# JuliaGraphics/Hikari.jl

Hardware: AMD Instinct MI355X
Metric: Mrays/s (higher is better)
Workload: dtype f32

## Files before the change

hikari.jl_amd/csrc/hk_ctx.cpp:

```cpp
#include "hk_host.h"

thread_local std::string g_err;
SlabCache g_slabs;

namespace hk {
static thread_local const Knobs* tl_knobs = nullptr;
const char* knob(const char* name) {
    if (!tl_knobs) return nullptr;
    auto it = tl_knobs->kv.find(name);
    return it == tl_knobs->kv.end() ? nullptr : it->second.c_str();
}
static const char* const KNOB_NAMES[] = {
    "HK_BATCH_PATHS_M", "HK_BVH_LEAF", "HK_BVH_BINS", "HK_QNODES", "HK_DEBUG_ALLOC", "HK_DELTA_ADVANCE", "HK_DYNAMIC_SEGMENTS", "HK_GREY", "HK_GREY_COMPACT", "HK_GREY_FLAT", "HK_MAX_PATHS_M",
    "HK_MID_LISTS", "HK_MID_PASS_PATHS_M", "HK_NODE_CACHE", "HK_NVDB_DENSE_MB", "HK_OVERLAP", "HK_PIPELINE", "HK_PIPELINE_AFTER", "HK_PIPELINE_MAX_PATHS_M", "HK_PRESELECT",
    "HK_SELECT_MIN_IDLE", "HK_SHADOW_FEED_ROUNDS", "HK_SHADOW_TRACK_BATCH", "HK_SMALL_PASS", "HK_SMALL_PASS_WAVES", "HK_SOBOL_LO_GB", "HK_SOBOL_TABLE_ONLY",
    "HK_STATE_CACHE_GB", "HK_STATE_SLAB", "HK_TICKET_SHARE", "HK_TRACK_ADVANCE", "HK_TRACK_EXTRA_ADVANCE", "HK_TRACK_MIN_PENDING", "HK_TRACK_POOL", "HK_TRACK_REFILL_IDLE",
    "HK_WALK_POOL", "HK_WALK_REFILL_IDLE", "HK_WALK_SPLIT", "HK_WAVES_PER_CU", "HK_READBACK_PIN", "HK_DEFER_EXTERNAL", "HK_SELECT_POOL", "HK_SMALL_PASS_FUSED", "HK_SMALL_PASS_MERGED", "HK_OCC_SCALE", "HK_ESCAPED_UNROLL", "HK_SHADOW_FINAL", "HK_TRI_PACK", "HK_LEAN_RECORDS", "HK_VIEW_CACHE", "HK_MAJORANT_BLOCK_VOXELS", "HK_BVH_BUILD_SMALL"};
static bool known_knob(const char* name) {
    for (const char* k : KNOB_NAMES)
        if (std::strcmp(k, name) == 0) return true;
    return false;
}
}
KnobScope::KnobScope(const hk::Knobs* k) : prev(hk::tl_knobs) { hk::tl_knobs = k; }
KnobScope::~KnobScope() { hk::tl_knobs = prev; }

void quiesce(hk_ctx* c) {
    if (!c) return;
    (void)hipStreamSynchronize(c->stream);
    if (c->aux) (void)hipStreamSynchronize(c->aux);
    for (auto& l : c->lanes)
        if (l.stream) (void)hipStreamSynchronize(l.stream);
}
int join_lanes(hk_ctx* c) {
    if (!c) return HK_OK;
    if (int e = flush_pending(c)) return e;
    if (!c->lanes_dirty) return HK_OK;
    for (auto& l : c->lanes)
        if (l.done) HIP_TRY(hipStreamWaitEvent(c->stream, l.done, 0));
    c->lanes_dirty = false;
    c->film_chain = false;
    if (c->have_span) HIP_TRY(hipEventRecord(c->ev_end, c->stream));
    return HK_OK;
}
hipEvent_t get_event(hk_ctx* c) {
    if (!c->event_pool.empty()) {
        hipEvent_t e = c->event_pool.back();
        c->event_pool.pop_back();
        return e;
    }
    hipEvent_t e;
    (void)hipEventCreate(&e);
    return e;
}
DCamera make_camera(const hk_camera& c) {
    DCamera d;
    std::memcpy(d.r2c, c.raster_to_camera, 64);
    std::memcpy(d.c2w, c.camera_to_world, 64);
    d.lens_radius = c.lens_radius;
    d.focal_distance = c.focal_distance;
    d.shutter_open = c.shutter_open;
    d.shutter_close = c.shutter_close;
    return d;
}

extern "C" const char* hk_last_error(void) { return g_err.c_str(); }

extern "C" int32_t hk_ctx_create(int32_t device_id, void* stream, hk_ctx** out) {
    if (!out) return fail(HK_ERR_INVALID, "out is null");
    int n = 0;
    HIP_TRY(hipGetDeviceCount(&n));
    if (device_id < 0 || device_id >= n) return fail(HK_ERR_INVALID, "bad device id");
    HIP_TRY(hipSetDevice(device_id));
    hk_ctx* c = new hk_ctx();
    c->device = device_id;
    c->stream = (hipStream_t)stream;
    hipDeviceProp_t prop;
    HIP_TRY(hipGetDeviceProperties(&prop, device_id));
    c->n_cu = prop.multiProcessorCount > 0 ? prop.multiProcessorCount : 256;
    c->own_stream_order = stream == nullptr;
    for (const char* name : hk::KNOB_NAMES)
        if (const char* e = std::getenv(name)) c->knobs.kv[name] = e;
    KnobScope knobs(&c->knobs);
    {
        c->waves_per_cu = hk::knob_int_in("HK_WAVES_PER_CU", 1, INT_MAX, 0);
        c->stat_rows = c->n_cu * 32 * 2;
        if (const char* e = hk::knob("HK_OVERLAP")) c->overlap = std::atoi(e) ? 1 : 0;
        else c->overlap = -1;
        if (const char* e = hk::knob("HK_STATE_CACHE_GB"))
            if (std::atol(e) >= 0) g_slabs.cap_bytes = (size_t)std::atol(e) << 30;
    }
    {
        std::vector<DStats> zero((size_t)c->stat_rows);
        std::memset(zero.data(), 0, zero.size() * sizeof(DStats));
        HIP_TRY(c->stats.upload(zero.data(), zero.size() * sizeof(DStats)));
    }
    HIP_TRY(hipEventCreate(&c->ev_begin));
    HIP_TRY(hipEventCreate(&c->ev_end));
    *out = c;
    return HK_OK;
// ... 266 lines not shown
```

hikari.jl_amd/csrc/hk_kernels.hip:

```cpp
#include <hip/hip_runtime.h>
#include <type_traits>
#include <cstdlib>
#include <cstdio>

#include "hikari_mi355x.h"
#include "hk_device.h"
#include "hk_edit_host.h"
#include "hk_bvh_decide.h"

using namespace hkd;

namespace {

__device__ __forceinline__ int lane_id() { return (int)(threadIdx.x & 63); }

struct WaveQ {
    uint32_t* base;
    int count;
};
__device__ __forceinline__ int global_wave() {
    const int w = (int)(threadIdx.x >> 6), b = (int)blockIdx.x;
    if (blockDim.x == 1024 && (gridDim.x & 7) == 0) return ((((b >> 3) * 4 + (w >> 2)) * 8 + (b & 7)) << 2) + (w & 3);
    if (blockDim.x == 512 && (gridDim.x & 7) == 0) return ((((b >> 3) * 2 + (w >> 2)) * 8 + (b & 7)) << 2) + (w & 3);
    return b * (int)(blockDim.x >> 6) + w;
// ... 2192 lines not shown
                        const int at = __popcll(dm & lt_mask);
                        pool[0][at] = e;
                        pool[1][at] = __float_as_uint(sp.x), pool[2][at] = __float_as_uint(sp.y), pool[3][at] = __float_as_uint(sp.z);
                        pool[4][at] = __float_as_uint(sn.x), pool[5][at] = __float_as_uint(sn.y), pool[6][at] = __float_as_uint(sn.z);
                        pool[7][at] = __float_as_uint(u_b);
                    }
                    pool_n = __popcll(dm);
                    __builtin_amdgcn_wave_barrier();
                }
            }
            const int avail = pool_n - pool_head;
            if (avail > 0) {
                const int rank = __popcll(free_m & lt_mask);
                if (!busy && rank < avail) {
                    const int at = pool_head + rank;
                    slot = pool[0][at];
                    p = mk3(__uint_as_float(pool[1][at]), __uint_as_float(pool[2][at]), __uint_as_float(pool[3][at]));
                    nn = mk3(__uint_as_float(pool[4][at]), __uint_as_float(pool[5][at]), __uint_as_float(pool[6][at]));
                    ub = __uint_as_float(pool[7][at]);
                    pmf = 1.0f - p_inf;
                    bits = root_bits, child = root_child;
                    lvl = 0;
                    busy = true;
                }
                const int free_n = __popcll(free_m);
                pool_head += free_n < avail ? free_n : avail;
            }
            if (__ballot(busy) == 0ull) {
                if (!more && pool_head == pool_n) break;
                continue;
            }
        }
        if (busy) {
            int res_light = -1;
            float res_pmf = 0.0f;
            if (lvl >= 64) {
                res_light = 0;
            } else {
                ++lvl;
                DLightNode n0, n1;
                if (NTOP > 0 && (int)child + 1 < n_top) {
                    n0 = lds_light_node<NTOP>(top, (int)child), n1 = lds_light_node<NTOP>(top, (int)child + 1);
                    asm volatile("" : "+v"(n0.bits));
                } else
                    n0 = load_light_node(sc.lnodes, (int)child), n1 = load_light_node(sc.lnodes, (int)child + 1);
                const float c0 = node_importance(n0, p, nn);
                const float c1 = node_importance(n1, p, nn);
                n_lnodes += 2;
                if (c0 == 0.0f && c1 == 0.0f) {
                    res_light = 0;
                } else {
                    const float p0 = c0 / (c0 + c1);
                    if (ub < p0) {
                        pmf *= p0;
                        ub = ub / p0;
                        bits = n0.bits, child = n0.child1_or_light;
                    } else {
                        pmf *= (1.0f - p0);
                        ub = (ub - p0) / (1.0f - p0);
                        bits = n1.bits, child = n1.child1_or_light;
                    }
                    if ((bits & 2u) && lvl < 64) {
                        res_light = (int)child;
                        res_pmf = pmf;
                    }
                }
            }
            if (res_light >= 0) {
                st.sel_light[slot] = make_uint2((uint32_t)res_light, __float_as_uint(res_pmf));
                busy = false;
            }
        }
    }
    stats += global_wave();
    wave_add(&stats->light_nodes, n_lnodes);
}

#ifndef HK_SHADE_WAVES_MATTE
#define HK_SHADE_WAVES_MATTE 4
#endif
#ifndef HK_SHADE_WAVES
#define HK_SHADE_WAVES 3
#endif
template <bool TWO_PLANES, bool SIMPLE>
HKD void shade_emission(const DPathState& st, const DPathGen& g, bool ones, const DScene& sc, const DTables& T, uint32_t slot, unsigned& n_lnodes, int depth, size_t seg) {
    const float4 H = st.hit[slot];
    const float4 O = ld_ray_o(st, g, slot, depth, seg), D = g.ray_d[slot];
    const v3 ro = mk3(O.x, O.y, O.z), rd = mk3(D.x, D.y, D.z);
    const float t_hit = H.x;
    const int prim = __float_as_int(H.y);
    const DTriMeta meta = tri_meta(sc, prim);
    if (meta.arealight <= 0) return;
    const Surface sf = surface_at(sc, prim, H.z, H.w, ro, rd, t_hit);
    const v3 wo = -rd;
    const uint2 pmeta = ld_meta(st, g, slot, depth);
    const S4 lambda = ld_lambda(st, g, slot, pmeta.y);
    const DLight& light = sc.lights[meta.arealight - 1];
    S4 Le = arealight_Le<TWO_PLANES, SIMPLE>(sc, T, light, wo, sf.n, sf.uv, lambda);
    if (is_black(Le)) return;
    const S4 beta = ld_throughput(g.beta, slot, ones), r_u = ld_ru(g, slot, ones, st.compact != 0), r_l = ld_rl(g, slot, ones, st.compact != 0);
    const uint32_t fl = pmeta.x;
    const int pdepth = (int)(fl & 0xff);
    const bool specular_bounce = (fl >> 8) & 1u;
    S4 contribution = beta * Le;
    S4 fin;
    if (pdepth == 0 || specular_bounce)
        fin = contribution / average(r_u);
    else {
        float choice = bvh_pmf(sc, sf.pi, sf.n, (int)meta.arealight, n_lnodes);
        float ct = fabsf(dot(sf.n, normalize(rd)));
        float light_pdf = 0.0f;
        if (ct > 0.0f && sf.area > 0.0f) light_pdf = choice * ((t_hit * t_hit) / (ct * sf.area));
        S4 rl = r_l * light_pdf;
        float den = average(r_u + rl);
        fin = den > 1e-10f ? contribution / den : contribution / average(r_u);
    }
    st4(&st.L[pmeta.y], ld4(&st.L[pmeta.y]) + fin);
}

template <int KIND>
struct ShadeWaves {
    static constexpr int value = (KIND == HK_MAT_COATED_DIFFUSE || KIND == HK_MAT_COATED_DIFFUSE_TRANSMISSION) ? 1 : (KIND == HK_MAT_MATTE ? HK_SHADE_WAVES_MATTE : HK_SHADE_WAVES);
};
#ifndef HK_SHADE_MIN_WAVES
#define HK_SHADE_MIN_WAVES 1
#endif
template <int KIND, bool SIMPLE, bool FT, bool PRE>
__device__ __forceinline__ void shade_body(const DPathState& st, const DScene& sc, const DTables& T, const DFrame& fr, const DSobol& sob, int depth, int first_kind, DStats* stats, const SegTickets& src,
                                           uint32_t* __restrict__ elist) {
    const int lane = lane_id();
    unsigned n_vertices = 0, n_lnodes = 0;
    HK_FOR_EACH_SEGMENT_FROM(gw, st, src) {
    const uint32_t* __restrict__ queue = st.mat_q + ((size_t)KIND * st.n_waves + gw) * st.wave_cap;
    const int n = *count_ptr(st, depth, Q_MAT0 + KIND, gw);
    const DPathGen g = gen_at(st, depth), gn = st.gen[(depth + 1) & 1];
    const size_t seg = (size_t)gw * st.wave_cap;
    const bool ones = depth == 0 && fr.implicit_ones;
    WavePos q_shadow{0}, q_next{0};
    if (!first_kind) {
        q_shadow.count = *count_ptr(st, depth, Q_SHADOW, gw);
        q_next.count = *count_ptr(st, depth + 1, Q_RAY, gw);
    }
    {
        int n_emit = 0;
        for (int base = 0; base < n || n_emit > 0; base += 64) {
            if (base < n) {
                const int i = base + lane;
                const uint32_t cand = i < n ? queue[i] : 0u;
                const bool em = i < n && (st.mat_id[cand] & HK_MAT_EMISSIVE_BIT) != 0;
                const unsigned long long m = __ballot(em);
                if (em) elist[n_emit + __popcll(m & ((1ull << lane) - 1ull))] = cand;
                n_emit += __popcll(m);
                if (n_emit < 64 && base + 64 < n) continue;
            }
            __builtin_amdgcn_fence(__ATOMIC_SEQ_CST, "wavefront");
            const int take = n_emit < 64 ? n_emit : 64;
            if (lane < take) shade_emission<KIND == HK_MAT_MATTE, SIMPLE>(st, g, ones, sc, T, elist[lane], n_lnodes, depth, seg);
            const int rest = n_emit - take;
            const uint32_t moved = lane < rest ? elist[64 + lane] : 0u;
            __builtin_amdgcn_fence(__ATOMIC_SEQ_CST, "wavefront");
            if (lane < rest) elist[lane] = moved;
            n_emit = rest;
        }
    }
    for (int base = 0; base < n; base += 64) {
        int i = base + lane;
        bool active = i < n;
        uint32_t slot = active ? queue[i] : 0u;
        bool push_shadow = false, push_ray = false;
        float4 H = make_float4(0, 0, 0, 0);
        Surface sf;
        v3 wo = mk3(0, 0, 1);
        DTriMeta meta{0u, 0u, 0u};
        S4 lambda = s4(0.0f), beta = s4(0.0f), r_u = s4(0.0f), kd_matte = s4(0.0f);
        uint32_t fl = 0, pslot = 0;
        int pdepth = 0, medium = -1;
        bool any_non_specular = false;
        SobolCtx sctx;
        const int base_dim = 6 + 7 * depth;
        float4 shO = make_float4(0, 0, 0, 0), shD = shO;
        S4 shLd = s4(0.0f), shRu = s4(0.0f), shRl = s4(0.0f);
        if (active) {
            ++n_vertices;
            H = stream_ld(&st.hit[slot]);
            float4 O = ld_ray_o(st, g, slot, depth, seg), D = stream_ld(&g.ray_d[slot]);
            v3 ro = mk3(O.x, O.y, O.z), rd = mk3(D.x, D.y, D.z);
            float t_hit = H.x;
            int prim = __float_as_int(H.y);
            sf = surface_at(sc, prim, H.z, H.w, ro, rd, t_hit);
            wo = -rd;
            meta = tri_meta(sc, prim);
            const uint2 pmeta = ld_meta(st, g, slot, depth);
            lambda = ld_lambda(st, g, slot, pmeta.y);
            if (ones)
                beta = s4(1.0f);
            else {
                const float4 bv = stream_ld(&g.beta[slot]);
                beta = s4(bv.x, bv.y, bv.z, bv.w);
            }
            r_u = ld_ru(g, slot, ones, st.compact != 0);
            fl = pmeta.x;
            pslot = pmeta.y;
            pdepth = (int)(fl & 0xff);
            any_non_specular = (fl >> 9) & 1u;
            medium = (int)(fl >> 16) - 1;

            int pix, k;
            split_slot(fr, pslot, pix, k);
            sctx = sobol_ctx_slot(sob, T.sobol, fr.x0, fr.y0, fr.tiles_x, pix, k, fr.first_sample + k * fr.sample_stride);

            if (KIND == HK_MAT_MATTE) kd_matte = matte_kd<SIMPLE>(sc, T, sc.materials[st.mat_id[slot] & ~HK_MAT_EMISSIVE_BIT], TexCtx(sf.uv, meta.prim_index, H.z, H.w), lambda);
#ifdef HK_ABLATE
            {
                float sink = 0.0f;
                if (HK_ABLATE == 1) {
                    uint32_t ps2 = pslot;
                    int d2 = base_dim;
                    asm volatile("" : "+v"(ps2));
                    asm volatile("" : "+s"(d2));
                    int pix2, k2;
                    split_slot(fr, ps2, pix2, k2);
                    SobolCtx c2 = sobol_ctx_slot(sob, T.sobol, fr.x0, fr.y0, fr.tiles_x, pix2, k2, fr.first_sample + k2 * fr.sample_stride);
                    v2 a = sobol_2d(c2, d2 + 3), b = sobol_2d(c2, d2 + 6);
                    sink = sobol_1d(c2, d2 + 1) + a.x + a.y + b.x + b.y + sobol_1d(c2, d2 + 7);
                }
                if (HK_ABLATE == 2 && sc.n_lights > 0) {
                    float u2 = H.z, pmf2;
                    asm volatile("" : "+v"(u2));
                    unsigned dummy = 0;
                    sink = (float)bvh_sample_light(sc, sf.pi, sf.ns, u2, pmf2, dummy) + pmf2;
                }
                if (HK_ABLATE == 3 && sc.n_lights > 0) {
                    uint32_t li = pslot;
                    asm volatile("" : "+v"(li));
                    LightSample l2 = sample_light(sc, T, sc.lights[li % (uint32_t)sc.n_lights], sf.pi, lambda, mk2(H.z, H.w));
                    sink = l2.pdf + l2.Li.x + l2.Li.w + l2.wi.x + l2.p_light.z;
                }
                if (HK_ABLATE == 4) {
                    S4 l2 = lambda;
                    asm volatile("" : "+v"(l2.x), "+v"(l2.y), "+v"(l2.z), "+v"(l2.w));
                    S4 k2 = matte_kd(sc, T, sc.materials[st.mat_id[slot] & ~HK_MAT_EMISSIVE_BIT], TexCtx(sf.uv, meta.prim_index, H.z, H.w), l2);
                    sink = k2.x + k2.y + k2.z + k2.w;
                }
                if (HK_ABLATE == 5) {
                    float b2 = H.z;
                    asm volatile("" : "+v"(b2));
                    Surface s2 = surface_at(sc, prim, b2, H.w, ro, rd, t_hit);
                    sink = s2.pi.x + s2.n.y + s2.ns.z + s2.uv.x + s2.area;
                }
                if (HK_ABLATE == 6) {
                    v3 w2 = wo;
                    asm volatile("" : "+v"(w2.x), "+v"(w2.y), "+v"(w2.z));
                    float p2;
                    S4 f2 = eval_matte_kd(kd_matte, w2, sf.n, sf.ns, p2);
                    BSDFSample s2 = sample_matte_kd(sc, sc.materials[st.mat_id[slot] & ~HK_MAT_EMISSIVE_BIT], kd_matte, w2, sf.ns, TexCtx(sf.uv, meta.prim_index, H.z, H.w), mk2(H.z, H.w));
                    sink = f2.x + f2.w + p2 + s2.pdf + s2.wi.x + s2.f.y;
                }
                asm volatile("" : : "v"(sink));
            }
#endif

            if (sc.n_lights > 0) {
                const DMaterial& mat = sc.materials[st.mat_id[slot] & ~HK_MAT_EMISSIVE_BIT];
                float light_pmf;
                int light_idx;
                if constexpr (PRE) {
                    const uint2 pre = st.sel_light[slot];
                    light_idx = (int)pre.x;
                    light_pmf = __uint_as_float(pre.y);
                } else {
                    float light_select = sobol_1d<FT>(sctx, base_dim + 1);
                    light_idx = bvh_sample_light(sc, sf.pi, sf.ns, light_select, light_pmf, n_lnodes);
                }
                if (light_idx >= 1 && light_idx <= sc.n_lights && light_pmf > 0.0f) {
                    const DLight& sel = sc.lights[light_idx - 1];
                    v2 u_light = mk2(0.0f, 0.0f);
                    if (sel.kind >= HK_LIGHT_AMBIENT) u_light = sobol_2d<FT>(sctx, base_dim + 3);
                    LightSample ls = sample_light<KIND == HK_MAT_MATTE, SIMPLE>(sc, T, sel, sf.pi, lambda, u_light);
                    if (ls.pdf > 0.0f && !is_black(ls.Li)) {
                        float bsdf_pdf;
                        S4 f = KIND == HK_MAT_MATTE ? eval_matte_kd(kd_matte, wo, ls.wi, sf.ns, bsdf_pdf)
                                                    : eval_bsdf<KIND>(sc, T, mat, wo, ls.wi, sf.ns, TexCtx(sf.uv, meta.prim_index, H.z, H.w), lambda, bsdf_pdf);
                        if (!is_black(f)) {
                            float ct = fabsf(dot(ls.wi, sf.ns));
                            S4 Ld = beta * f * ls.Li * ct;
                            if (!is_black(Ld)) {
                                v3 off = 1e-4f * sf.ns;
                                v3 so = dot(ls.wi, sf.ns) > 0.0f ? sf.pi + off : sf.pi - off;
                                v3 tl = ls.p_light - so;
                                float tmax = sqrtf(dot(tl, tl)) - 1e-3f;
                                float nbp = ls.is_delta ? 0.0f : bsdf_pdf;
                                shO = make_float4(so.x, so.y, so.z, tmax);
                                shD = make_float4(ls.wi.x, ls.wi.y, ls.wi.z, __int_as_float(medium));
                                shLd = Ld;
                                shRu = r_u * nbp;
                                shRl = (r_u * ls.pdf) * light_pmf;
                                push_shadow = true;
                            }
                        }
                    }
                }
            }
        }
        {
            const size_t ps = seg + (size_t)wp_push(q_shadow, push_shadow);
            if (push_shadow && st.sh_final) {
                const S4 mis = s4(shRu.x) * s4(1.0f) + s4(shRl.x) * s4(1.0f);
                shD.w = average(mis);
                stream_st(&st.sh_o[ps], shO);
                stream_st(&st.sh_d[ps], shD);
                stream_st(&st.sh_Ld[ps], shLd);
                stream_st(&st.sh_slot[ps], pslot);
            } else if (push_shadow) {
                stream_st(&st.sh_o[ps], shO);
                stream_st(&st.sh_d[ps], shD);
                stream_st(&st.sh_Ld[ps], shLd);
                if (st.compact) {
#if HK_NT
                    __builtin_nontemporal_store((hk_f2){shRu.x, shRl.x}, (hk_f2*)(reinterpret_cast<float2*>(st.sh_ru) + ps));
#else
                    reinterpret_cast<float2*>(st.sh_ru)[ps] = make_float2(shRu.x, shRl.x);
#endif
                } else
                    st_shadow_weights(st, ps, shRu, shRl);
                stream_st(&st.sh_slot[ps], pslot);
            }
        }
        float4 nO = make_float4(0, 0, 0, 0), nD = nO;
        S4 nb = s4(0.0f), nrl = s4(0.0f);
        uint32_t nflags = 0;
        if (active) {
            int new_depth = pdepth + 1;
            if (new_depth < fr.max_depth) {
                const DMaterial& mat = sc.materials[st.mat_id[slot] & ~HK_MAT_EMISSIVE_BIT];
                const DMediumInterface mi = sc.mis[meta.mi];
                float uc = (KIND == HK_MAT_GLASS || KIND > HK_MAT_CONDUCTOR) && KIND != HK_MAT_FALLBACK ? sobol_1d<FT>(sctx, base_dim + 4) : 0.0f;
                v2 u = (KIND == HK_MAT_MIRROR || KIND == HK_MAT_GLASS || KIND == HK_MAT_THIN_DIELECTRIC) ? mk2(0.0f, 0.0f) : sobol_2d<FT>(sctx, base_dim + 6);
                bool regularize = fr.regularize && any_non_specular;
                BSDFSample s = KIND == HK_MAT_MATTE ? sample_matte_kd<SIMPLE>(sc, mat, kd_matte, wo, sf.ns, TexCtx(sf.uv, meta.prim_index, H.z, H.w), u)
                                                    : sample_bsdf<KIND>(sc, T, mat, wo, sf.ns, TexCtx(sf.uv, meta.prim_index, H.z, H.w), lambda, u, uc, regularize);
                if (s.pdf > 0.0f && !is_black(s.f)) {
                    float ct = fabsf(dot(s.wi, sf.ns));
                    nb = s.is_specular ? beta * s.f : beta * s.f * ct / s.pdf;
                    nrl = s.is_specular ? r_u : r_u / s.pdf;
                    bool cont = true;
                    if (new_depth > 3) {
                        float rr = sobol_1d<FT>(sctx, base_dim + 7);
                        float q = maxf(0.05f, 1.0f - max_component(nb));
                        if (rr < q)
                            cont = false;
                        else
                            nb = nb * (1.0f / (1.0f - q));
                    }
                    if (cont) {
                        int new_medium = (mi.inside != mi.outside) ? (dot(s.wi, sf.n) > 0.0f ? mi.outside : mi.inside) : medium;
                        v3 off = dot(s.wi, sf.n) > 0.0f ? sf.n : -sf.n;
                        v3 no = sf.pi + off * 0.0001f;
                        nO = make_float4(no.x, no.y, no.z, INF_F);
                        nD = make_float4(s.wi.x, s.wi.y, s.wi.z, 0.0f);
                        bool ans = any_non_specular || !s.is_specular;
                        nflags = (uint32_t)new_depth | ((s.is_specular ? 1u : 0u) << 8) | ((ans ? 1u : 0u) << 9) | ((uint32_t)(new_medium + 1) << 16);
                        push_ray = true;
                    }
                }
            }
        }
        {
            const size_t pn = seg + (size_t)wp_push(q_next, push_ray);
            if (push_ray) {
                stream_st(&gn.ray_o[pn], nO);
                if (st.compact) nD.w = nrl.x;
                stream_st(&gn.ray_d[pn], nD);
                stream_st(&gn.beta[pn], nb);
                st_ru_rl(gn, pn, r_u, nrl, st.compact != 0);
                st_lambda(gn, pn, lambda);
                st_meta(st, gn, pn, nflags, pslot);
            }
        }
    }
    if (lane == 0) {
        *count_ptr(st, depth, Q_SHADOW, gw) = q_shadow.count;
        *count_ptr(st, depth + 1, Q_RAY, gw) = q_next.count;
    }
    }
    stats += global_wave();
    wave_add(&stats->vertices, n_vertices);
    wave_add(&stats->light_nodes, n_lnodes);
}
template <int KIND, bool SIMPLE = false, bool FT = false, bool PRE = false>
__global__ void __attribute__((amdgpu_flat_work_group_size(256, 256), amdgpu_waves_per_eu(ShadeWaves<KIND>::value))) k_shade(DPathState st, DScene sc, DTables T, DFrame fr, DSobol sob, int depth, int first_kind, DStats* stats) {
    __shared__ uint32_t emit_list[4 * 128];
    shade_body<KIND, SIMPLE, FT, PRE>(st, sc, T, fr, sob, depth, first_kind, stats, seg_open(st, ticket_ptr(st, depth, TK_SHADE0 + KIND), st.dynamic_segments != 0, depth, Q_MAT0 + KIND),
                                      emit_list + (threadIdx.x >> 6) * 128);
}

template <class W> HKD W wone();
template <> HKD float wone<float>() { return 1.0f; }
template <> HKD S4 wone<S4>() { return s4(1.0f); }
HKD S4 wide(S4 v) { return v; }
HKD S4 wide(float v) { return s4(v); }
HKD bool is_black(float v) { return v == 0.0f; }
template <bool COMPACT>
HKD void shadow_contribute(const DPathState& st, uint32_t rec, S4 T_ray, S4 tr_u, S4 tr_l) {
    if (is_black(T_ray)) return;
    S4 w_u, w_l;
    ld_shadow_weights<COMPACT>(st, rec, w_u, w_l);
    S4 mis = w_u * tr_u + w_l * tr_l;
    float den = average(mis);
    if (den > 1e-10f) {
        S4 fin = ld4(&st.sh_Ld[rec]) * T_ray / den;
        if (!is_black(fin)) {
            const uint32_t pslot = st.sh_slot[rec];
            st4(&st.L[pslot], ld4(&st.L[pslot]) + fin);
        }
    }
}

HKD void shadow_contribute_final(const DPathState& st, uint32_t rec, float den) {
    if (den > 1e-10f) {
        const S4 fin = ld4(&st.sh_Ld[rec]) * s4(1.0f) / den;
        if (!is_black(fin)) {
            const uint32_t pslot = st.sh_slot[rec];
            st4(&st.L[pslot], ld4(&st.L[pslot]) + fin);
        }
    }
}
HKD void shadow_contribute_rt(const DPathState& st, uint32_t rec, S4 T_ray, S4 tr_u, S4 tr_l) {
    if (st.compact)
        shadow_contribute<true>(st, rec, T_ray, tr_u, tr_l);
    else
        shadow_contribute<false>(st, rec, T_ray, tr_u, tr_l);
}

template <bool COUNT, int NC, bool QN = false>
__device__ __forceinline__ void shadow_body(const DPathState& st, const DScene& sc, int depth, DStats* stats, SegStream stream, int* __restrict__ stack, const NodeCache& cache) {
    const int lane = lane_id();
    const unsigned long long lt_mask = (1ull << lane) - 1ull;
    const int DONE = (int)0x80000000;
    unsigned n_nodes = 0, n_tris = 0, n_casts = 0, n_hits = 0;
    HK_DBG_DECL
    uint32_t seg = 0;
    int n = 0, cursor = 0;
    bool more = true;
    bool have = false;
    uint32_t slot = 0;
    float rec_den = 0.0f;
    LaneRay r;
    r.cur = r.pend = DONE;
    for (;;) {
        const unsigned long long run_m = __ballot(have && r.cur != DONE);
        if (run_m == 0ull || (64 - __popcll(run_m) >= HK_TRACE_MIN_IDLE && (cursor < n || more))) {
            if (have && r.cur == DONE) {
                if (r.best.prim < 0) {
                    if (st.sh_final)
                        shadow_contribute_final(st, slot, rec_den);
                    else
                        shadow_contribute<true>(st, slot, s4(1.0f), s4(1.0f), s4(1.0f));
                } else
                    ++n_hits;
                have = false;
            }
            while (more && cursor >= n) {
                const int gw = stream_next(stream, st.n_waves);
                if (gw >= st.n_waves) {
                    more = false;
                    break;
                }
                seg = (uint32_t)gw * (uint32_t)st.wave_cap;
                n = *count_ptr(st, depth, Q_SHADOW, gw);
                cursor = 0;
            }
            const unsigned long long want = __ballot(!have);
            const int avail = n - cursor;
            const int rank = __popcll(want & lt_mask);
            if (!have && rank < avail) {
                slot = seg + (uint32_t)(cursor + rank);
// ... 2115 lines not shown
```

hikari.jl_amd/csrc/hk_launch_impl.h:

```cpp
#pragma once
#include "hk_launch.h"

namespace hk {

template <bool V>
using bool_c = std::bool_constant<V>;
template <int V>
using int_c = std::integral_constant<int, V>;
template <class F>
static void with_bool(bool b, F&& f) {
    if (b) f(bool_c<true>{});
    else f(bool_c<false>{});
}
template <int V0, int... Vs, class F>
static void with_int(int v, F&& f) {
    if constexpr (sizeof...(Vs) == 0) f(int_c<V0>{});
    else if (v == V0) f(int_c<V0>{});
    else with_int<Vs...>(v, f);
}

#ifndef HK_OCC_SCALE_DEFAULT
#define HK_OCC_SCALE_DEFAULT 1.0f
#endif
static inline int grid_for(int n, int block, int cap) {
// ... 139 lines not shown
    if (lean_scene(sc)) {
        lean_dispatch<HK_SHADOW_BLOCK16, HK_SHADOW_NC16, HK_SHADOW_NC32>(sc, fr, [&](auto COUNT, auto STACK, auto BLOCK, auto NC, auto QN) {
            constexpr int block = decltype(BLOCK)::value;
            launch_resident<k_shadow<decltype(COUNT)::value, decltype(STACK)::value, block, decltype(NC)::value, decltype(QN)::value>>(s, n_cu, st, block, 8, sc, depth, stats);
        });
        return;
    }
    const int mc = sc.n_media > 0 ? media_mask_class(sc) : 0;
    const bool split = sc.all_grey && grey_mode() && walk_split_mode() && sc.bvh_depth <= 16 && st.wq_a != nullptr;
    with_bool(fr.count_nodes != 0, [&](auto COUNT) {
        constexpr bool c = decltype(COUNT)::value;
        if (split && mc == 8) launch_walk_split<c, 8>(s, n_cu, st, sc, fr, depth, stats);
        else if (split && mc == 2) launch_walk_split<c, 2>(s, n_cu, st, sc, fr, depth, stats);
        else with_int<0, 1, 2, 4, 8, 15>(mc, [&](auto MM) { launch_shadow_walk<c, decltype(MM)::value>(s, n_cu, st, sc, T, fr, depth, stats); });
    });
}
void launch_segment_lists(hipStream_t s, const DPathState& st, int n, const int* depths, const int* queues) {
    if (n <= 0) return;
    SegQueues qs;
    qs.n = n;
    for (int i = 0; i < n; ++i) {
        qs.depth[i] = depths[i];
        qs.q[i] = queues[i];
    }
    hipLaunchKernelGGL(k_segment_lists, dim3(n, HK_LIST_SPLIT), dim3(1024), 0, s, st, qs);
}
void launch_medium(hipStream_t s, int n_cu, const DPathState& st, const DScene& sc, const DTables& T, const DFrame& fr, const DSobol& sob, int depth, DStats* stats) {
    {
        const int d = depth, q = Q_MEDIUM;
        launch_segment_lists(s, st, 1, &d, &q);
    }
    const bool grey = sc.all_grey && grey_mode();
    const bool flat = grey && grey_flat_mode();
    const bool pool = flat && track_pool_mode() && sc.grey_pool;
    auto track = [&](auto MM, auto GREY) { launch_resident<k_track<decltype(MM)::value, decltype(GREY)::value>>(s, n_cu, st, 256, 8, sc, T, fr, depth, stats, sc.media); };
    auto track_flat = [&](auto MM, auto BRICKS) {
        constexpr int mm = decltype(MM)::value;
        constexpr bool bricks = decltype(BRICKS)::value;
        if (pool) launch_resident<k_track_pool<mm, bricks>>(s, n_cu, st, 256, 8, sc, fr, depth, stats, sc.media);
        else launch_resident<k_track_flat<mm, bricks>>(s, n_cu, st, 256, 8, sc, fr, depth, stats, sc.media);
    };
    switch (media_mask_class(sc)) {
        case 1: track(int_c<1>{}, bool_c<false>{}); break;
        case 2:
            if (flat) track_flat(int_c<2>{}, bool_c<false>{});
            else with_bool(grey, [&](auto GREY) { track(int_c<2>{}, GREY); });
            break;
        case 4: track(int_c<4>{}, bool_c<false>{}); break;
        case 8:
            if (flat) with_bool(sc.grey_bricks != 0, [&](auto BRICKS) { track_flat(int_c<8>{}, BRICKS); });
            else with_bool(grey, [&](auto GREY) { track(int_c<8>{}, GREY); });
            break;
        default: track(int_c<15>{}, bool_c<false>{}); break;
    }
    {
        const int d = depth, q = Q_SCATTER;
        launch_segment_lists(s, st, 1, &d, &q);
    }
    with_bool(sobol_tables_cover(sob, depth), [&](auto FT) { launch_resident<k_scatter<decltype(FT)::value>>(s, n_cu, st, 256, 8, sc, T, fr, sob, depth, stats); });
}
void launch_detect_camera_medium(hipStream_t s, const DPathState& st, const DScene& sc, float x, float y, float z, DStats* stats) {
    hipLaunchKernelGGL(k_detect_camera_medium, dim3(1), dim3(64), 0, s, st, sc, x, y, z, stats);
}
void launch_escaped(hipStream_t s, int n_cu, const DPathState& st, const DScene& sc, const DTables& T, const DFrame& fr, int depth) {
    with_bool(knob_int("HK_ESCAPED_UNROLL", 1) != 2, [&](auto ONE) { launch_resident<k_escaped<decltype(ONE)::value ? 1 : 2>>(s, n_cu, st, 256, 8, sc, T, depth, fr.implicit_ones); });
}
bool preselect_lights(const DScene& sc, const DPathState& st) {
    return sc.n_media == 0 && sc.num_bvh_lights >= HK_PRESELECT_MIN && st.sel_light != nullptr && knob_on("HK_PRESELECT");
}
void launch_light_select(hipStream_t s, int n_cu, const DPathState& st, const DScene& sc, const DTables& T, const DFrame& fr, const DSobol& sob, int depth, uint32_t kinds_mask, DStats* stats) {
    const int min_idle = knob_int_in("HK_SELECT_MIN_IDLE", 1, 64, HK_SELECT_MIN_IDLE);
    const bool pool = knob_on("HK_SELECT_POOL");
    with_bool(sobol_tables_cover(sob, depth), [&](auto FT) {
        constexpr bool ft = decltype(FT)::value;
        if (pool) launch_resident<k_light_select_pool<ft>>(s, n_cu, st, HK_SELECT_BLOCK, 8, sc, T, fr, sob, depth, kinds_mask, stats);
        else launch_resident<k_light_select<ft>>(s, n_cu, st, 256, 8, sc, T, fr, sob, depth, kinds_mask, min_idle, stats);
    });
}
void launch_shade(hipStream_t s, int n_cu, int kind, const DPathState& st, const DScene& sc, const DTables& T, const DFrame& fr, const DSobol& sob, int depth, int first_kind, DStats* stats) {
    auto shade = [&](auto KIND, auto SIMPLE, auto FT, auto PRE) {
        launch_resident<k_shade<decltype(KIND)::value, decltype(SIMPLE)::value, decltype(FT)::value, decltype(PRE)::value>>(s, n_cu, st, 256, 8, sc, T, fr, sob, depth, first_kind, stats);
    };
    const bool ft = sobol_tables_cover(sob, depth);
    const bool light_kind = kind == HK_MAT_MATTE || kind == HK_MAT_MIRROR || kind == HK_MAT_GLASS || kind == HK_MAT_CONDUCTOR;
    if (light_kind && preselect_lights(sc, st))
        with_int<HK_MAT_MATTE, HK_MAT_MIRROR, HK_MAT_GLASS, HK_MAT_CONDUCTOR>(kind, [&](auto KIND) { with_bool(ft, [&](auto FT) { shade(KIND, bool_c<false>{}, FT, bool_c<true>{}); }); });
    else if (kind == HK_MAT_MATTE && sc.simple_lights)
        with_bool(ft, [&](auto FT) { shade(int_c<HK_MAT_MATTE>{}, bool_c<true>{}, FT, bool_c<false>{}); });
    else if (light_kind && ft)
        with_int<HK_MAT_MATTE, HK_MAT_MIRROR, HK_MAT_GLASS, HK_MAT_CONDUCTOR>(kind, [&](auto KIND) { shade(KIND, bool_c<false>{}, bool_c<true>{}, bool_c<false>{}); });
    else
        with_int<HK_MAT_MATTE, HK_MAT_MIRROR, HK_MAT_GLASS, HK_MAT_CONDUCTOR, HK_MAT_COATED_DIFFUSE, HK_MAT_THIN_DIELECTRIC, HK_MAT_DIFFUSE_TRANSMISSION, HK_MAT_COATED_DIFFUSE_TRANSMISSION,
                 HK_MAT_COATED_CONDUCTOR, HK_MAT_FALLBACK>(kind, [&](auto KIND) { shade(KIND, bool_c<false>{}, bool_c<false>{}, bool_c<false>{}); });
}
#ifndef HK_SMALL_PASS_NC
#define HK_SMALL_PASS_NC 1536
#endif
static int small_pass_class(const DScene& sc, uint32_t kinds_mask) {
    const int mode = knob_int("HK_SMALL_PASS_FUSED", 2);
    if (mode == 0) return 0;
    if (!(lean_scene(sc) && sc.bvh_depth <= HK_LDS_STACK && node_cache_on())) return 0;
    if (kinds_mask == (1u << HK_MAT_MATTE) && sc.simple_lights && !sc.has_escape_lights && sc.bvh_depth <= 16 && sc.num_bvh_lights < HK_PRESELECT_MIN) return 1;
    const uint32_t light_kinds = (1u << HK_MAT_MATTE) | (1u << HK_MAT_MIRROR) | (1u << HK_MAT_GLASS) | (1u << HK_MAT_CONDUCTOR);
    return (mode >= 2 && kinds_mask != 0 && (kinds_mask & ~light_kinds) == 0) ? 2 : 0;
}
bool small_pass_fusable(const DScene& sc, uint32_t kinds_mask) { return small_pass_class(sc, kinds_mask) != 0; }
template <int BLOCK, bool GENERAL, int STACK, class... A>
static bool small_pass_blocks(hipStream_t s, int n_cu, const DPathState& st, bool dry, A&&... args) {
    constexpr auto kernel = k_small_pass<HK_SMALL_PASS_NC, BLOCK, GENERAL, STACK>;
    int blocks = cached_blocks<kernel>(BLOCK, n_cu, 1);
    if (blocks * (BLOCK / 64) > st.n_waves) blocks = st.n_waves / (BLOCK / 64);
    if (blocks < 1) return false;
    if (!dry) hipLaunchKernelGGL(kernel, dim3(blocks), dim3(BLOCK), 0, s, st, args...);
    return true;
}
bool launch_small_pass(hipStream_t s, int n_cu, const DPathState& st, const DScene& sc, const DTables& T, const DFrame& fr, const DFilter& flt, const DCamera& cam, const DSobol& sob, int max_depth,
                       uint32_t kinds_mask, DStats* stats, bool dry, void* accum, int film_mode) {
    const int cls = small_pass_class(sc, kinds_mask);
    if (cls == 0 || !st.small_pass || st.dynamic_segments || fr.count_nodes) return false;
    if (((long)st.capacity + 63) / 64 / 16 > 4L * n_cu) return false;
    for (int depth = 0; depth < max_depth; ++depth)
        if (sobol_tables_cover(sob, depth)) return false;
    const int merged = knob_on("HK_SMALL_PASS_MERGED") ? 1 : 0;
    if (st.n_waves > 8 * n_cu) return false;
    bool launched = false;
    auto pass = [&](auto GENERAL, auto STACK) {
        with_bool(st.n_waves > 4 * n_cu, [&](auto WIDE) {
            launched = small_pass_blocks<decltype(WIDE)::value ? 512 : 256, decltype(GENERAL)::value, decltype(STACK)::value>(s, n_cu, st, dry, sc, T, fr, flt, cam, sob, max_depth, sc.n_lights > 0 ? 1 : 0, merged,
                                                                                                                       accum, film_mode, kinds_mask, stats);
        });
    };
    if (cls == 2 && sc.bvh_depth > 16) pass(bool_c<true>{}, int_c<HK_LDS_STACK>{});
    else if (cls == 2) pass(bool_c<true>{}, int_c<16>{});
    else pass(bool_c<false>{}, int_c<16>{});
    return launched;
}
void launch_film(hipStream_t s, const DPathState& st, const DFrame& fr, const DTables& T, void* accum, bool f64) {
    int g = grid_for(fr.n_pixels_padded >> 6, 4, 4096);
    if (f64)
        hipLaunchKernelGGL(k_film<double>, dim3(g), dim3(256), 0, s, st, fr, T, (double*)accum);
    else
        hipLaunchKernelGGL(k_film<float>, dim3(g), dim3(256), 0, s, st, fr, T, (float*)accum);
}
void launch_sobol_table(hipStream_t s, const DSobol& sob, const DFrame& fr, uint2* table, int rows) {
    hipLaunchKernelGGL(k_sobol_table, dim3(grid_for((long)rows * fr.n_pixels_padded > 0x3fffffff ? 0x3fffffff : rows * fr.n_pixels_padded, 256, 8192)), dim3(256), 0, s, sob, fr, table, rows);
}
void launch_sobol_lo_table(hipStream_t s, const DSobol& sob, const DFrame& fr, uint16_t* table, int rows, int base, int stride, int count) {
    hipLaunchKernelGGL(k_sobol_lo_table, dim3(65536), dim3(256), 0, s, sob, fr, table, rows, base, stride, count);
}
template <class Layout>
void launch_finalize(hipStream_t s, const void* accum, bool f64, Layout out, int w, int h) {
    int g = grid_for(w * h, 256, 4096);
    if (f64)
        hipLaunchKernelGGL((k_finalize<double, Layout>), dim3(g), dim3(256), 0, s, (const double*)accum, out, w, h);
    else
        hipLaunchKernelGGL((k_finalize<float, Layout>), dim3(g), dim3(256), 0, s, (const float*)accum, out, w, h);
}
template <class Layout>
void launch_aux(hipStream_t s, const DScene& sc, const DCamera& cam, int h, int w, float miss_depth, float* albedo, Layout out) {
    hipLaunchKernelGGL(k_aux<Layout>, dim3(grid_for(h * w, HK_TRACE_BLOCK, 2048)), dim3(HK_TRACE_BLOCK), 0, s, sc, cam, h, w, miss_depth, albedo, out);
}
template <class Layout>
void launch_variance(hipStream_t s, Layout src, float* variance, int h, int w) {
    hipLaunchKernelGGL(k_variance<Layout>, dim3(grid_for(h * w, 256, 8192)), dim3(256), 0, s, src, variance, h, w);
}
template <class Layout>
// ... 84 lines not shown
```

Baseline: 10030.

## Add lean Matte shade kernel variant with LDS stash and scalar MIS weights

Adds a LEAN specialization of the Matte shade kernel for simple-light lean scenes with compact 32-bit metadata. It replaces the per-wavelength r_u/r_l vectors with scalars, packs path flags into one meta word, and spills surface normal, wo, kd, beta and meta into a shared-memory stash across the light-sampling call so fewer values stay live in registers. It also forces segment indices and counts to be wave-uniform via readfirstlane and raises the waves-per-EU hint. The path is gated behind the HK_SHADE_LEAN knob, and it assumes uniform r_u and no media.

Measured after the change: 10460, median of 6. 4.3% higher.

```diff
diff --git a/hikari.jl_amd/csrc/hk_ctx.cpp b/hikari.jl_amd/csrc/hk_ctx.cpp
--- a/hikari.jl_amd/csrc/hk_ctx.cpp
+++ b/hikari.jl_amd/csrc/hk_ctx.cpp
@@ -15,7 +15,7 @@
     "HK_MID_LISTS", "HK_MID_PASS_PATHS_M", "HK_NODE_CACHE", "HK_NVDB_DENSE_MB", "HK_OVERLAP", "HK_PIPELINE", "HK_PIPELINE_AFTER", "HK_PIPELINE_MAX_PATHS_M", "HK_PRESELECT",
     "HK_SELECT_MIN_IDLE", "HK_SHADOW_FEED_ROUNDS", "HK_SHADOW_TRACK_BATCH", "HK_SMALL_PASS", "HK_SMALL_PASS_WAVES", "HK_SOBOL_LO_GB", "HK_SOBOL_TABLE_ONLY",
     "HK_STATE_CACHE_GB", "HK_STATE_SLAB", "HK_TICKET_SHARE", "HK_TRACK_ADVANCE", "HK_TRACK_EXTRA_ADVANCE", "HK_TRACK_MIN_PENDING", "HK_TRACK_POOL", "HK_TRACK_REFILL_IDLE",
-    "HK_WALK_POOL", "HK_WALK_REFILL_IDLE", "HK_WALK_SPLIT", "HK_WAVES_PER_CU", "HK_READBACK_PIN", "HK_DEFER_EXTERNAL", "HK_SELECT_POOL", "HK_SMALL_PASS_FUSED", "HK_SMALL_PASS_MERGED", "HK_OCC_SCALE", "HK_ESCAPED_UNROLL", "HK_SHADOW_FINAL", "HK_TRI_PACK", "HK_LEAN_RECORDS", "HK_VIEW_CACHE", "HK_MAJORANT_BLOCK_VOXELS", "HK_BVH_BUILD_SMALL"};
+    "HK_WALK_POOL", "HK_WALK_REFILL_IDLE", "HK_WALK_SPLIT", "HK_WAVES_PER_CU", "HK_READBACK_PIN", "HK_DEFER_EXTERNAL", "HK_SELECT_POOL", "HK_SMALL_PASS_FUSED", "HK_SMALL_PASS_MERGED", "HK_OCC_SCALE", "HK_ESCAPED_UNROLL", "HK_SHADOW_FINAL", "HK_TRI_PACK", "HK_LEAN_RECORDS", "HK_VIEW_CACHE", "HK_MAJORANT_BLOCK_VOXELS", "HK_BVH_BUILD_SMALL", "HK_SHADE_LEAN"};
 static bool known_knob(const char* name) {
     for (const char* k : KNOB_NAMES)
         if (std::strcmp(k, name) == 0) return true;
diff --git a/hikari.jl_amd/csrc/hk_kernels.hip b/hikari.jl_amd/csrc/hk_kernels.hip
--- a/hikari.jl_amd/csrc/hk_kernels.hip
+++ b/hikari.jl_amd/csrc/hk_kernels.hip
@@ -2298,7 +2298,13 @@
 #ifndef HK_SHADE_WAVES
 #define HK_SHADE_WAVES 3
 #endif
-template <bool TWO_PLANES, bool SIMPLE>
+#ifndef HK_SHADE_WAVES_LEAN
+#define HK_SHADE_WAVES_LEAN 5
+#endif
+#ifndef HK_SHADE_WAVES_LEAN_HASH
+#define HK_SHADE_WAVES_LEAN_HASH 5
+#endif
+template <bool TWO_PLANES, bool SIMPLE, bool LEAN = false>
 HKD void shade_emission(const DPathState& st, const DPathGen& g, bool ones, const DScene& sc, const DTables& T, uint32_t slot, unsigned& n_lnodes, int depth, size_t seg) {
     const float4 H = st.hit[slot];
     const float4 O = ld_ray_o(st, g, slot, depth, seg), D = g.ray_d[slot];
@@ -2309,27 +2315,47 @@
     if (meta.arealight <= 0) return;
     const Surface sf = surface_at(sc, prim, H.z, H.w, ro, rd, t_hit);
     const v3 wo = -rd;
-    const uint2 pmeta = ld_meta(st, g, slot, depth);
+    uint2 pmeta;
+    if constexpr (LEAN) {
+        const uint32_t w = reinterpret_cast<const uint32_t*>(g.meta)[slot];
+        pmeta = make_uint2((uint32_t)depth | (((w >> 30) & 1u) << 8), w & 0x3fffffffu);
+    } else
+        pmeta = ld_meta(st, g, slot, depth);
     const S4 lambda = ld_lambda(st, g, slot, pmeta.y);
     const DLight& light = sc.lights[meta.arealight - 1];
     S4 Le = arealight_Le<TWO_PLANES, SIMPLE>(sc, T, light, wo, sf.n, sf.uv, lambda);
     if (is_black(Le)) return;
-    const S4 beta = ld_throughput(g.beta, slot, ones), r_u = ld_ru(g, slot, ones, st.compact != 0), r_l = ld_rl(g, slot, ones, st.compact != 0);
+    const S4 beta = ld_throughput(g.beta, slot, ones);
     const uint32_t fl = pmeta.x;
     const int pdepth = (int)(fl & 0xff);
     const bool specular_bounce = (fl >> 8) & 1u;
     S4 contribution = beta * Le;
     S4 fin;
-    if (pdepth == 0 || specular_bounce)
-        fin = contribution / average(r_u);
-    else {
-        float choice = bvh_pmf(sc, sf.pi, sf.n, (int)meta.arealight, n_lnodes);
-        float ct = fabsf(dot(sf.n, normalize(rd)));
-        float light_pdf = 0.0f;
-        if (ct > 0.0f && sf.area > 0.0f) light_pdf = choice * ((t_hit * t_hit) / (ct * sf.area));
-        S4 rl = r_l * light_pdf;
-        float den = average(r_u + rl);
-        fin = den > 1e-10f ? contribution / den : contribution / average(r_u);
+    if constexpr (LEAN) {
+        fin = contribution;
+        if (!(pdepth == 0 || specular_bounce)) {
+            const float r_l = ones ? 1.0f : D.w;
+            float choice = bvh_pmf(sc, sf.pi, sf.n, (int)meta.arealight, n_lnodes);
+            float ct = fabsf(dot(sf.n, normalize(rd)));
+            float light_pdf = 0.0f;
+            if (ct > 0.0f && sf.area > 0.0f) light_pdf = choice * ((t_hit * t_hit) / (ct * sf.area));
+            const float a = 1.0f + r_l * light_pdf;
+            const float den = (((a + a) + a) + a) / 4.0f;
+            if (den > 1e-10f) fin = contribution / den;
+        }
+    } else {
+        const S4 r_u = ld_ru(g, slot, ones, st.compact != 0), r_l = ld_rl(g, slot, ones, st.compact != 0);
+        if (pdepth == 0 || specular_bounce)
+            fin = contribution / average(r_u);
+        else {
+            float choice = bvh_pmf(sc, sf.pi, sf.n, (int)meta.arealight, n_lnodes);
+            float ct = fabsf(dot(sf.n, normalize(rd)));
+            float light_pdf = 0.0f;
+            if (ct > 0.0f && sf.area > 0.0f) light_pdf = choice * ((t_hit * t_hit) / (ct * sf.area));
+            S4 rl = r_l * light_pdf;
+            float den = average(r_u + rl);
+            fin = den > 1e-10f ? contribution / den : contribution / average(r_u);
+        }
     }
     st4(&st.L[pmeta.y], ld4(&st.L[pmeta.y]) + fin);
 }
@@ -2341,21 +2367,35 @@
 #ifndef HK_SHADE_MIN_WAVES
 #define HK_SHADE_MIN_WAVES 1
 #endif
-template <int KIND, bool SIMPLE, bool FT, bool PRE>
+#define HK_SHADE_STASH 16
+template <int KIND, bool SIMPLE, bool FT, bool PRE, bool LEAN = false>
 __device__ __forceinline__ void shade_body(const DPathState& st, const DScene& sc, const DTables& T, const DFrame& fr, const DSobol& sob, int depth, int first_kind, DStats* stats, const SegTickets& src,
-                                           uint32_t* __restrict__ elist) {
+                                           uint32_t* __restrict__ elist,
+                                           float* stash = nullptr) {
+    static_assert(!LEAN || (KIND == HK_MAT_MATTE && HK_LAMBDA_BY_SLOT), "the lean body is Matte's");
     const int lane = lane_id();
     unsigned n_vertices = 0, n_lnodes = 0;
-    HK_FOR_EACH_SEGMENT_FROM(gw, st, src) {
+    unsigned nv_wave = 0;
+    unsigned* const nl_stash = LEAN ? reinterpret_cast<unsigned*>(stash) + (HK_SHADE_STASH - 1) * 256 + threadIdx.x : nullptr;
+    auto nl_flush = [&]() {
+        if constexpr (LEAN) {
+            if (n_lnodes) *nl_stash += n_lnodes;
+            n_lnodes = 0;
+        }
+    };
+    if constexpr (LEAN) *nl_stash = 0u;
+    auto uni = [](int v) { return LEAN ? __builtin_amdgcn_readfirstlane(v) : v; };
+    HK_FOR_EACH_SEGMENT_FROM(gw_v, st, src) {
+    const int gw = uni(gw_v);
     const uint32_t* __restrict__ queue = st.mat_q + ((size_t)KIND * st.n_waves + gw) * st.wave_cap;
-    const int n = *count_ptr(st, depth, Q_MAT0 + KIND, gw);
+    const int n = uni(*count_ptr(st, depth, Q_MAT0 + KIND, gw));
     const DPathGen g = gen_at(st, depth), gn = st.gen[(depth + 1) & 1];
     const size_t seg = (size_t)gw * st.wave_cap;
     const bool ones = depth == 0 && fr.implicit_ones;
     WavePos q_shadow{0}, q_next{0};
     if (!first_kind) {
-        q_shadow.count = *count_ptr(st, depth, Q_SHADOW, gw);
-        q_next.count = *count_ptr(st, depth + 1, Q_RAY, gw);
+        q_shadow.count = uni(*count_ptr(st, depth, Q_SHADOW, gw));
+        q_next.count = uni(*count_ptr(st, depth + 1, Q_RAY, gw));
     }
     {
         int n_emit = 0;
@@ -2371,7 +2411,8 @@
             }
             __builtin_amdgcn_fence(__ATOMIC_SEQ_CST, "wavefront");
             const int take = n_emit < 64 ? n_emit : 64;
-            if (lane < take) shade_emission<KIND == HK_MAT_MATTE, SIMPLE>(st, g, ones, sc, T, elist[lane], n_lnodes, depth, seg);
+            if (lane < take) shade_emission<KIND == HK_MAT_MATTE, SIMPLE, LEAN>(st, g, ones, sc, T, elist[lane], n_lnodes, depth, seg);
+            nl_flush();
             const int rest = n_emit - take;
             const uint32_t moved = lane < rest ? elist[64 + lane] : 0u;
             __builtin_amdgcn_fence(__ATOMIC_SEQ_CST, "wavefront");
@@ -2393,11 +2434,19 @@
         int pdepth = 0, medium = -1;
         bool any_non_specular = false;
         SobolCtx sctx;
+        using W = std::conditional_t<LEAN, float, S4>;
+        auto stash_at = [&]() {
+            int i = (int)threadIdx.x;
+            asm volatile("" : "+v"(i));
+            return stash + i;
+        };
         const int base_dim = 6 + 7 * depth;
         float4 shO = make_float4(0, 0, 0, 0), shD = shO;
-        S4 shLd = s4(0.0f), shRu = s4(0.0f), shRl = s4(0.0f);
+        S4 shLd = s4(0.0f);
+        W shRu{}, shRl{};
+        if constexpr (LEAN) nv_wave += (unsigned)(n - base < 64 ? n - base : 64);
         if (active) {
-            ++n_vertices;
+            if constexpr (!LEAN) ++n_vertices;
             H = stream_ld(&st.hit[slot]);
             float4 O = ld_ray_o(st, g, slot, depth, seg), D = stream_ld(&g.ray_d[slot]);
             v3 ro = mk3(O.x, O.y, O.z), rd = mk3(D.x, D.y, D.z);
@@ -2406,20 +2455,28 @@
             sf = surface_at(sc, prim, H.z, H.w, ro, rd, t_hit);
             wo = -rd;
             meta = tri_meta(sc, prim);
-            const uint2 pmeta = ld_meta(st, g, slot, depth);
-            lambda = ld_lambda(st, g, slot, pmeta.y);
+            uint32_t meta_w = 0;
+            if constexpr (LEAN) {
+                meta_w = reinterpret_cast<const uint32_t*>(g.meta)[slot];
+                pslot = meta_w & 0x3fffffffu;
+                pdepth = depth;
+                any_non_specular = (meta_w >> 31) != 0u;
+            } else {
+                const uint2 pmeta = ld_meta(st, g, slot, depth);
+                fl = pmeta.x;
+                pslot = pmeta.y;
+                pdepth = (int)(fl & 0xff);
+                any_non_specular = (fl >> 9) & 1u;
+                medium = (int)(fl >> 16) - 1;
+                r_u = ld_ru(g, slot, ones, st.compact != 0);
+            }
+            lambda = ld_lambda(st, g, slot, pslot);
             if (ones)
                 beta = s4(1.0f);
             else {
                 const float4 bv = stream_ld(&g.beta[slot]);
                 beta = s4(bv.x, bv.y, bv.z, bv.w);
             }
-            r_u = ld_ru(g, slot, ones, st.compact != 0);
-            fl = pmeta.x;
-            pslot = pmeta.y;
-            pdepth = (int)(fl & 0xff);
-            any_non_specular = (fl >> 9) & 1u;
-            medium = (int)(fl >> 16) - 1;
 
             int pix, k;
             split_slot(fr, pslot, pix, k);
@@ -2476,6 +2533,14 @@
             }
 #endif
 
+            if constexpr (LEAN) {
+                float* sp = stash + threadIdx.x;
+                sp[0 * 256] = sf.n.x, sp[1 * 256] = sf.n.y, sp[2 * 256] = sf.n.z;
+                sp[3 * 256] = wo.x, sp[4 * 256] = wo.y, sp[5 * 256] = wo.z;
+                sp[6 * 256] = kd_matte.x, sp[7 * 256] = kd_matte.y, sp[8 * 256] = kd_matte.z, sp[9 * 256] = kd_matte.w;
+                sp[10 * 256] = beta.x, sp[11 * 256] = beta.y, sp[12 * 256] = beta.z, sp[13 * 256] = beta.w;
+                sp[14 * 256] = __uint_as_float(meta_w);
+            }
             if (sc.n_lights > 0) {
                 const DMaterial& mat = sc.materials[st.mat_id[slot] & ~HK_MAT_EMISSIVE_BIT];
                 float light_pmf;
@@ -2495,6 +2560,12 @@
                     LightSample ls = sample_light<KIND == HK_MAT_MATTE, SIMPLE>(sc, T, sel, sf.pi, lambda, u_light);
                     if (ls.pdf > 0.0f && !is_black(ls.Li)) {
                         float bsdf_pdf;
+                        if constexpr (LEAN) {
+                            const float* sp = stash_at();
+                            wo = mk3(sp[3 * 256], sp[4 * 256], sp[5 * 256]);
+                            kd_matte = s4(sp[6 * 256], sp[7 * 256], sp[8 * 256], sp[9 * 256]);
+                            beta = s4(sp[10 * 256], sp[11 * 256], sp[12 * 256], sp[13 * 256]);
+                        }
                         S4 f = KIND == HK_MAT_MATTE ? eval_matte_kd(kd_matte, wo, ls.wi, sf.ns, bsdf_pdf)
                                                     : eval_bsdf<KIND>(sc, T, mat, wo, ls.wi, sf.ns, TexCtx(sf.uv, meta.prim_index, H.z, H.w), lambda, bsdf_pdf);
                         if (!is_black(f)) {
@@ -2509,8 +2580,13 @@
                                 shO = make_float4(so.x, so.y, so.z, tmax);
                                 shD = make_float4(ls.wi.x, ls.wi.y, ls.wi.z, __int_as_float(medium));
                                 shLd = Ld;
-                                shRu = r_u * nbp;
-                                shRl = (r_u * ls.pdf) * light_pmf;
+                                if constexpr (LEAN) {
+                                    shRu = nbp;
+                                    shRl = ls.pdf * light_pmf;
+                                } else {
+                                    shRu = r_u * nbp;
+                                    shRl = (r_u * ls.pdf) * light_pmf;
+                                }
                                 push_shadow = true;
                             }
                         }
@@ -2518,9 +2594,19 @@
                 }
             }
         }
+        nl_flush();
         {
             const size_t ps = seg + (size_t)wp_push(q_shadow, push_shadow);
-            if (push_shadow && st.sh_final) {
+            if constexpr (LEAN) {
+                if (push_shadow) {
+                    const float m = shRu + shRl;
+                    shD.w = (((m + m) + m) + m) / 4.0f;
+                    stream_st(&st.sh_o[ps], shO);
+                    stream_st(&st.sh_d[ps], shD);
+                    stream_st(&st.sh_Ld[ps], shLd);
+                    stream_st(&st.sh_slot[ps], pslot);
+                }
+            } else if (push_shadow && st.sh_final) {
                 const S4 mis = s4(shRu.x) * s4(1.0f) + s4(shRl.x) * s4(1.0f);
                 shD.w = average(mis);
                 stream_st(&st.sh_o[ps], shO);
@@ -2543,13 +2629,28 @@
             }
         }
         float4 nO = make_float4(0, 0, 0, 0), nD = nO;
-        S4 nb = s4(0.0f), nrl = s4(0.0f);
+        S4 nb = s4(0.0f);
+        W nrl{};
         uint32_t nflags = 0;
         if (active) {
             int new_depth = pdepth + 1;
             if (new_depth < fr.max_depth) {
                 const DMaterial& mat = sc.materials[st.mat_id[slot] & ~HK_MAT_EMISSIVE_BIT];
-                const DMediumInterface mi = sc.mis[meta.mi];
+                DMediumInterface mi{};
+                if constexpr (LEAN) {
+                    const float* sp = stash_at();
+                    sf.n = mk3(sp[0 * 256], sp[1 * 256], sp[2 * 256]);
+                    wo = mk3(sp[3 * 256], sp[4 * 256], sp[5 * 256]);
+                    kd_matte = s4(sp[6 * 256], sp[7 * 256], sp[8 * 256], sp[9 * 256]);
+                    beta = s4(sp[10 * 256], sp[11 * 256], sp[12 * 256], sp[13 * 256]);
+                    const uint32_t meta_w = __float_as_uint(sp[14 * 256]);
+                    pslot = meta_w & 0x3fffffffu;
+                    any_non_specular = (meta_w >> 31) != 0u;
+                    int pix, k;
+                    split_slot(fr, pslot, pix, k);
+                    sctx = sobol_ctx_slot(sob, T.sobol, fr.x0, fr.y0, fr.tiles_x, pix, k, fr.first_sample + k * fr.sample_stride);
+                } else
+                    mi = sc.mis[meta.mi];
                 float uc = (KIND == HK_MAT_GLASS || KIND > HK_MAT_CONDUCTOR) && KIND != HK_MAT_FALLBACK ? sobol_1d<FT>(sctx, base_dim + 4) : 0.0f;
                 v2 u = (KIND == HK_MAT_MIRROR || KIND == HK_MAT_GLASS || KIND == HK_MAT_THIN_DIELECTRIC) ? mk2(0.0f, 0.0f) : sobol_2d<FT>(sctx, base_dim + 6);
                 bool regularize = fr.regularize && any_non_specular;
@@ -2558,7 +2659,8 @@
                 if (s.pdf > 0.0f && !is_black(s.f)) {
                     float ct = fabsf(dot(s.wi, sf.ns));
                     nb = s.is_specular ? beta * s.f : beta * s.f * ct / s.pdf;
-                    nrl = s.is_specular ? r_u : r_u / s.pdf;
+                    if constexpr (LEAN) nrl = s.is_specular ? 1.0f : 1.0f / s.pdf;
+                    else nrl = s.is_specular ? r_u : r_u / s.pdf;
                     bool cont = true;
                     if (new_depth > 3) {
                         float rr = sobol_1d<FT>(sctx, base_dim + 7);
@@ -2569,7 +2671,8 @@
                             nb = nb * (1.0f / (1.0f - q));
                     }
                     if (cont) {
-                        int new_medium = (mi.inside != mi.outside) ? (dot(s.wi, sf.n) > 0.0f ? mi.outside : mi.inside) : medium;
+                        int new_medium = -1;
+                        if constexpr (!LEAN) new_medium = (mi.inside != mi.outside) ? (dot(s.wi, sf.n) > 0.0f ? mi.outside : mi.inside) : medium;
                         v3 off = dot(s.wi, sf.n) > 0.0f ? sf.n : -sf.n;
                         v3 no = sf.pi + off * 0.0001f;
                         nO = make_float4(no.x, no.y, no.z, INF_F);
@@ -2583,7 +2686,15 @@
         }
         {
             const size_t pn = seg + (size_t)wp_push(q_next, push_ray);
-            if (push_ray) {
+            if constexpr (LEAN) {
+                if (push_ray) {
+                    stream_st(&gn.ray_o[pn], nO);
+                    nD.w = nrl;
+                    stream_st(&gn.ray_d[pn], nD);
+                    stream_st(&gn.beta[pn], nb);
+                    stream_st(reinterpret_cast<uint32_t*>(gn.meta) + pn, pslot | (((nflags >> 8) & 1u) << 30) | (((nflags >> 9) & 1u) << 31));
+                }
+            } else if (push_ray) {
                 stream_st(&gn.ray_o[pn], nO);
                 if (st.compact) nD.w = nrl.x;
                 stream_st(&gn.ray_d[pn], nD);
@@ -2599,15 +2710,24 @@
         *count_ptr(st, depth + 1, Q_RAY, gw) = q_next.count;
     }
     }
+    if constexpr (LEAN) {
+        n_vertices = lane == 0 ? nv_wave : 0u;
+        n_lnodes = *nl_stash;
+    }
     stats += global_wave();
     wave_add(&stats->vertices, n_vertices);
     wave_add(&stats->light_nodes, n_lnodes);
 }
-template <int KIND, bool SIMPLE = false, bool FT = false, bool PRE = false>
-__global__ void __attribute__((amdgpu_flat_work_group_size(256, 256), amdgpu_waves_per_eu(ShadeWaves<KIND>::value))) k_shade(DPathState st, DScene sc, DTables T, DFrame fr, DSobol sob, int depth, int first_kind, DStats* stats) {
+template <int KIND, bool SIMPLE = false, bool FT = false, bool PRE = false, bool LEAN = false>
+__global__ void __attribute__((amdgpu_flat_work_group_size(256, 256), amdgpu_waves_per_eu(LEAN ? (FT ? HK_SHADE_WAVES_LEAN : HK_SHADE_WAVES_LEAN_HASH) : ShadeWaves<KIND>::value))) k_shade(DPathState st, DScene sc, DTables T, DFrame fr, DSobol sob, int depth, int first_kind, DStats* stats) {
     __shared__ uint32_t emit_list[4 * 128];
-    shade_body<KIND, SIMPLE, FT, PRE>(st, sc, T, fr, sob, depth, first_kind, stats, seg_open(st, ticket_ptr(st, depth, TK_SHADE0 + KIND), st.dynamic_segments != 0, depth, Q_MAT0 + KIND),
-                                      emit_list + (threadIdx.x >> 6) * 128);
+    SegTickets src = seg_open(st, ticket_ptr(st, depth, TK_SHADE0 + KIND), st.dynamic_segments != 0, depth, Q_MAT0 + KIND);
+    if constexpr (LEAN) {
+        src.pos = __builtin_amdgcn_readfirstlane(src.pos), src.k0 = __builtin_amdgcn_readfirstlane(src.k0);
+        __shared__ float stash[HK_SHADE_STASH * 256];
+        shade_body<KIND, SIMPLE, FT, PRE, true>(st, sc, T, fr, sob, depth, first_kind, stats, src, emit_list + (threadIdx.x >> 6) * 128, stash);
+    } else
+        shade_body<KIND, SIMPLE, FT, PRE>(st, sc, T, fr, sob, depth, first_kind, stats, src, emit_list + (threadIdx.x >> 6) * 128);
 }
 
 template <class W> HKD W wone();
diff --git a/hikari.jl_amd/csrc/hk_launch_impl.h b/hikari.jl_amd/csrc/hk_launch_impl.h
--- a/hikari.jl_amd/csrc/hk_launch_impl.h
+++ b/hikari.jl_amd/csrc/hk_launch_impl.h
@@ -245,6 +245,10 @@
         launch_resident<k_shade<decltype(KIND)::value, decltype(SIMPLE)::value, decltype(FT)::value, decltype(PRE)::value>>(s, n_cu, st, 256, 8, sc, T, fr, sob, depth, first_kind, stats);
     };
     const bool ft = sobol_tables_cover(sob, depth);
+    if (kind == HK_MAT_MATTE && sc.simple_lights && lean_scene(sc) && st.compact && st.meta32 && st.sh_final && !preselect_lights(sc, st) && knob_on("HK_SHADE_LEAN")) {
+        with_bool(ft, [&](auto FT) { launch_resident<k_shade<HK_MAT_MATTE, true, decltype(FT)::value, false, true>>(s, n_cu, st, 256, 8, sc, T, fr, sob, depth, first_kind, stats); });
+        return;
+    }
     const bool light_kind = kind == HK_MAT_MATTE || kind == HK_MAT_MIRROR || kind == HK_MAT_GLASS || kind == HK_MAT_CONDUCTOR;
     if (light_kind && preselect_lights(sc, st))
         with_int<HK_MAT_MATTE, HK_MAT_MIRROR, HK_MAT_GLASS, HK_MAT_CONDUCTOR>(kind, [&](auto KIND) { with_bool(ft, [&](auto FT) { shade(KIND, bool_c<false>{}, FT, bool_c<true>{}); }); });
```
